# jhtonyKoo/music_mixing_style_transfer

Hardware: AMD Instinct MI355X
Metric: stereo 44.1 kHz segments/sec (FXencoder+MixFXcloner fwd) (higher is better)
Workload: dtype bf16

## Files before the change

include/mst_hip.h:

```cpp
#ifndef MST_HIP_H
#define MST_HIP_H

#include <stddef.h>
#include <stdint.h>

#ifdef __cplusplus
extern "C" {
#endif

typedef enum {
    MST_OK = 0,
    MST_ERR_ARG = -1,
    MST_ERR_UNSUPPORTED = -2,
    MST_ERR_HIP = -3,
    MST_ERR_STATE = -4,
    MST_ERR_WORKSPACE = -5
} MstStatus;

typedef enum {
    MST_PREC_F32 = 0,
    MST_PREC_BF16 = 1,
    MST_PREC_BF16X3 = 2
} MstPrecision;

#define MST_MAX_BLOCKS 32

int mst_version(void);
const char *mst_last_error(void);

typedef struct MstTcn MstTcn;

typedef struct {
    int nblocks;
    int ninputs;
    int noutputs;
    int channels;
    int kernel_size;
    int cond_dim;
    int dilations[MST_MAX_BLOCKS];
    int causal;
} MstTcnDesc;

int mst_tcn_create(const MstTcnDesc *desc, MstTcn **out);
int mst_tcn_destroy(MstTcn *tcn);

int mst_tcn_load_block(MstTcn *tcn, int n, const float *conv_w, const float *bn_weight, const float *bn_bias,
                       const float *bn_mean, const float *bn_var, float bn_eps, const float *film_w,
                       const float *film_b, const float *res_w, void *stream);
int mst_tcn_load_output(MstTcn *tcn, const float *w, const float *b, void *stream);

int mst_tcn_set_cond(MstTcn *tcn, const float *cond_dev, int n_rows, long block_stride, void *stream);

size_t mst_tcn_workspace_bytes(const MstTcn *tcn, int B, int L, int precision);

int mst_tcn_forward(MstTcn *tcn, const float *x_dev, float *y_dev, int B, int L, int precision,
                    void *workspace, size_t workspace_bytes, void *stream);
int mst_tcn_forward_blocks(MstTcn *tcn, const float *x_dev, float *act_dev, int B, int L, int precision, int n_run,
                           void *workspace, size_t workspace_bytes, void *stream);

int mst_tcn_set_tuning(MstTcn *tcn, int flags);
int mst_tcn_get_tuning(const MstTcn *tcn, int *flags, int *last_forward_fused_block0);

int mst_tcn_timing_begin(MstTcn *tcn, int max_forwards);
int mst_tcn_timing_end(MstTcn *tcn, float *ms_out, int *n_forwards);

int mst_calib_mainloop(int launches, float *ms_per_launch, float *sclk_mhz, void *stream);

typedef struct MstEnc MstEnc;

typedef struct {
    int nblocks;
    int channels[MST_MAX_BLOCKS + 1];
    int kernels[MST_MAX_BLOCKS];
    int strides[MST_MAX_BLOCKS];
    int dilations[MST_MAX_BLOCKS];
    int valid_padding;
    float act_slope;
} MstEncDesc;

int mst_enc_create(const MstEncDesc *desc, MstEnc **out);
int mst_enc_destroy(MstEnc *enc);
int mst_enc_load_conv(MstEnc *enc, int block, int which, const float *w, const float *bias,
                      const float *bn_weight, const float *bn_bias, const float *bn_mean, const float *bn_var,
                      float bn_eps, void *stream);
int mst_enc_set_tuning(MstEnc *enc, long rows_min_tiles);
int mst_enc_set_schedule(MstEnc *enc, int flags);
int mst_global_avgpool(const float *x_dev, float *y_dev, long rows, int L, void *stream);
int mst_enc_zero_stuff(const float *x_dev, float *y_dev, long rows, long L, int stride, long pad_left, long Lu, void *stream);
size_t mst_enc_workspace_bytes(const MstEnc *enc, int B, int L);
int mst_enc_forward(MstEnc *enc, const float *x_dev, float *emb_dev, int B, int L, int precision, void *workspace,
                    size_t workspace_bytes, void *stream);
int mst_enc_forward_blocks(MstEnc *enc, const float *x_dev, float *out_dev, int B, int L, int precision, int n_run,
                           void *workspace, size_t workspace_bytes, void *stream);
int mst_enc_conv_length(const MstEnc *enc, int block, int which, int L);
int mst_enc_forward_conv(MstEnc *enc, int block, int which, const float *x_dev, float *y_dev, int B, int L, void *stream);
int mst_enc_block_length(const MstEnc *enc, int block, int L);

int mst_film_forward(const float *w_dev, const float *b_dev, const float *cond_dev, int rows, int cond_dim, int C,
                     const float *x_dev, float *y_dev, int B, long L, float *table_dev, void *stream);

int mst_embedding_mean(const float *emb_dev, int n_rows, int dim, float *out_dev, void *stream);

#define MST_SUMSQ_SLOTS 64
#define MST_FX_FORM_EQ_LANE_APPLY 1
#define MST_FX_FORM_EQ_VALU_ENDS 2
#define MST_FX_FORM_COMP_SLICE_SMALL 4
typedef struct {
    unsigned struct_size;
    int forms;
    const double *in_scale_dev;
    double *out_sumsq_dev;
    const double *in_sumsq_dev;
    int post_rms;
    float post_gain;
// ... 150 lines not shown
```

music_mixing_style_transfer_amd/_lib.py:

```python
import ctypes as C
import os

import torch

_HERE = os.path.dirname(os.path.abspath(__file__))
LIB_PATH = os.path.join(_HERE, "csrc", "libmst_hip.so")

MST_OK = 0
MST_PREC_F32 = 0
MST_PREC_BF16 = 1
MST_PREC_BF16X3 = 2
MST_MAX_BLOCKS = 32
TCN_TUNING_DEFAULT = 245
PRECISIONS = {"fp32": MST_PREC_F32, "f32": MST_PREC_F32, "bf16": MST_PREC_BF16, "bf16x3": MST_PREC_BF16X3}

STATUS_NAMES = {0: "MST_OK", -1: "MST_ERR_ARG", -2: "MST_ERR_UNSUPPORTED", -3: "MST_ERR_HIP", -4: "MST_ERR_STATE",
                -5: "MST_ERR_WORKSPACE"}


class MstTcnDesc(C.Structure):
    _fields_ = [("nblocks", C.c_int), ("ninputs", C.c_int), ("noutputs", C.c_int), ("channels", C.c_int),
                ("kernel_size", C.c_int), ("cond_dim", C.c_int), ("dilations", C.c_int * MST_MAX_BLOCKS), ("causal", C.c_int)]


FX_FORM_EQ_LANE_APPLY, FX_FORM_EQ_VALU_ENDS, FX_FORM_COMP_SLICE_SMALL = 1, 2, 4


class MstFxFuse(C.Structure):
    _fields_ = [("struct_size", C.c_uint), ("forms", C.c_int), ("in_scale_dev", C.c_void_p), ("out_sumsq_dev", C.c_void_p),
                ("in_sumsq_dev", C.c_void_p), ("post_rms", C.c_int), ("post_gain", C.c_float), ("out_in_sumsq_dev", C.c_void_p),
                ("out_ms_dev", C.c_void_p), ("in_ms_dev", C.c_void_p)]

    def __init__(self, in_scale_dev=None, out_sumsq_dev=None, in_sumsq_dev=None, post_rms=0, post_gain=0.0, out_in_sumsq_dev=None,
                 out_ms_dev=None, in_ms_dev=None, forms=0):
        super().__init__(C.sizeof(MstFxFuse), forms, in_scale_dev, out_sumsq_dev, in_sumsq_dev, post_rms, post_gain, out_in_sumsq_dev,
                         out_ms_dev, in_ms_dev)


FX_COMP_SPLIT_SERIAL, FX_COMP_TIME_PARALLEL, FX_COMP_WAVE_SERIAL = 0, 1, 2


class MstFxBiquadItemsPlan(C.Structure):
    _fields_ = [("struct_size", C.c_uint), ("M", C.c_int), ("tables_offset", C.c_size_t), ("item_stride", C.c_size_t), ("powers_offset", C.c_size_t),
                ("coef_offset", C.c_size_t), ("total_bytes", C.c_size_t)]

    def __init__(self, *a, **kw):
        super().__init__(*a, **kw)
        self.struct_size = C.sizeof(MstFxBiquadItemsPlan)


class MstFxBiquadPlan(C.Structure):
    _fields_ = [("struct_size", C.c_uint), ("time_parallel", C.c_int), ("M", C.c_int), ("scan_threads", C.c_int), ("record_doubles", C.c_int),
                ("nchunks", C.c_long), ("ends_offset", C.c_size_t), ("starts_offset", C.c_size_t)]

    def __init__(self):
        super().__init__(C.sizeof(MstFxBiquadPlan))


class MstFxCompressorPlan(C.Structure):
    _fields_ = [("struct_size", C.c_uint), ("form", C.c_int), ("nslices", C.c_int), ("record_doubles", C.c_int), ("nchunks", C.c_long),
                ("nbatch", C.c_long), ("ntiles", C.c_long), ("kappa", C.c_double), ("kappa_limit", C.c_double), ("xl_offset", C.c_size_t),
                ("maps_offset", C.c_size_t), ("ystart_offset", C.c_size_t), ("tab_offset", C.c_size_t), ("carry_offset", C.c_size_t),
                ("tsums_offset", C.c_size_t), ("total_bytes", C.c_size_t)]

    def __init__(self):
        super().__init__(C.sizeof(MstFxCompressorPlan))


class MstEncDesc(C.Structure):
    _fields_ = [("nblocks", C.c_int), ("channels", C.c_int * (MST_MAX_BLOCKS + 1)), ("kernels", C.c_int * MST_MAX_BLOCKS),
                ("strides", C.c_int * MST_MAX_BLOCKS), ("dilations", C.c_int * MST_MAX_BLOCKS), ("valid_padding", C.c_int), ("act_slope", C.c_float)]


MST_MSS_MAX_SCALES = 8
MSS_MODES = {"midside": 0, "ori": 1}
MSS_WINDOWS = {"hann": 0, "hamming": 1}


class MstMssDesc(C.Structure):
    _fields_ = [("struct_size", C.c_uint), ("mode", C.c_int), ("n_scales", C.c_int), ("n_fft", C.c_int * MST_MSS_MAX_SCALES),
                ("hop", C.c_int * MST_MSS_MAX_SCALES), ("win_length", C.c_int * MST_MSS_MAX_SCALES), ("window", C.c_int),
                ("eps", C.c_double)]

    def __init__(self, mode=0, n_fft=(), hop=(), win_length=(), window=0, eps=1e-7):
        super().__init__()
        self.struct_size, self.mode, self.n_scales, self.window, self.eps = C.sizeof(MstMssDesc), mode, len(n_fft), window, eps
        for i in range(min(len(n_fft), MST_MSS_MAX_SCALES)):
            self.n_fft[i], self.hop[i], self.win_length[i] = n_fft[i], hop[i], win_length[i]


_P = C.c_void_p
_F = C.c_void_p

SIGNATURES = {
    "mst_version": (C.c_int, []),
    "mst_last_error": (C.c_char_p, []),
    "mst_tcn_create": (C.c_int, [C.POINTER(MstTcnDesc), C.POINTER(_P)]),
    "mst_tcn_destroy": (C.c_int, [_P]),
    "mst_tcn_load_block": (C.c_int, [_P, C.c_int, _F, _F, _F, _F, _F, C.c_float, _F, _F, _F, _P]),
    "mst_tcn_load_output": (C.c_int, [_P, _F, _F, _P]),
    "mst_tcn_set_cond": (C.c_int, [_P, _F, C.c_int, C.c_long, _P]),
    "mst_tcn_workspace_bytes": (C.c_size_t, [_P, C.c_int, C.c_int, C.c_int]),
    "mst_tcn_forward": (C.c_int, [_P, _F, _F, C.c_int, C.c_int, C.c_int, _P, C.c_size_t, _P]),
    "mst_tcn_forward_blocks": (C.c_int, [_P, _F, _F, C.c_int, C.c_int, C.c_int, C.c_int, _P, C.c_size_t, _P]),
    "mst_tcn_set_tuning": (C.c_int, [_P, C.c_int]),
    "mst_tcn_get_tuning": (C.c_int, [_P, C.POINTER(C.c_int), C.POINTER(C.c_int)]),
    "mst_tcn_timing_begin": (C.c_int, [_P, C.c_int]),
    "mst_tcn_timing_end": (C.c_int, [_P, C.POINTER(C.c_float), C.POINTER(C.c_int)]),
    "mst_calib_mainloop": (C.c_int, [C.c_int, C.POINTER(C.c_float), C.POINTER(C.c_float), _P]),
    "mst_enc_create": (C.c_int, [C.POINTER(MstEncDesc), C.POINTER(_P)]),
    "mst_enc_destroy": (C.c_int, [_P]),
    "mst_enc_load_conv": (C.c_int, [_P, C.c_int, C.c_int, _F, _F, _F, _F, _F, _F, C.c_float, _P]),
    "mst_enc_set_tuning": (C.c_int, [_P, C.c_long]),
    "mst_enc_set_schedule": (C.c_int, [_P, C.c_int]),
    "mst_global_avgpool": (C.c_int, [_F, _F, C.c_long, C.c_int, _P]),
    "mst_enc_zero_stuff": (C.c_int, [_F, _F, C.c_long, C.c_long, C.c_int, C.c_long, C.c_long, _P]),
    "mst_enc_workspace_bytes": (C.c_size_t, [_P, C.c_int, C.c_int]),
    "mst_enc_forward": (C.c_int, [_P, _F, _F, C.c_int, C.c_int, C.c_int, _P, C.c_size_t, _P]),
    "mst_enc_forward_blocks": (C.c_int, [_P, _F, _F, C.c_int, C.c_int, C.c_int, C.c_int, _P, C.c_size_t, _P]),
    "mst_enc_block_length": (C.c_int, [_P, C.c_int, C.c_int]),
    "mst_enc_conv_length": (C.c_int, [_P, C.c_int, C.c_int, C.c_int]),
    "mst_enc_forward_conv": (C.c_int, [_P, C.c_int, C.c_int, _F, _F, C.c_int, C.c_int, _P]),
    "mst_film_forward": (C.c_int, [_F, _F, _F, C.c_int, C.c_int, C.c_int, _F, _F, C.c_int, C.c_long, _F, _P]),
    "mst_embedding_mean": (C.c_int, [_F, C.c_int, C.c_int, _F, _P]),
    "mst_fx_biquad_scratch_bytes": (C.c_size_t, [C.c_int, C.c_long, C.c_int, C.c_int]),
    "mst_fx_biquad_plan": (C.c_int, [C.c_int, C.c_long, C.c_int, C.c_int, C.POINTER(MstFxBiquadPlan)]),
    "mst_fx_biquad_tables": (C.c_int, [C.POINTER(C.c_double), C.c_int, C.c_int, C.POINTER(C.c_double), C.POINTER(C.c_double)]),
    "mst_fx_compressor_plan": (C.c_int, [C.c_int, C.c_long, C.c_int, C.c_double, C.c_double, C.c_double, C.c_int, C.POINTER(MstFxCompressorPlan)]),
    "mst_fx_biquad_cascade": (C.c_int, [_F, _F, C.c_int, C.c_long, C.c_int, C.POINTER(C.c_double), C.c_int, _P, C.c_size_t, _P, _P]),
    "mst_fx_biquad_items_scratch_bytes": (C.c_size_t, [C.c_int, C.c_long, C.c_int, C.c_int]),
    "mst_fx_biquad_items_plan": (C.c_int, [C.c_int, C.c_long, C.c_int, C.c_int, C.POINTER(MstFxBiquadItemsPlan)]),
    "mst_fx_biquad_cascade_items": (C.c_int, [_F, _F, C.c_int, C.c_long, C.c_int, _P, C.c_int, _P, C.c_size_t, _P, _P]),
    "mst_fx_compressor_items_table_bytes": (C.c_size_t, [C.c_int]),
    "mst_fx_compressor_items_prepare": (C.c_int, [_P, C.c_int, C.c_long, C.c_int, C.c_double, C.c_int, _P, C.c_size_t, C.POINTER(C.c_int)]),
    "mst_fx_compressor_items": (C.c_int, [_F, _F, C.c_int, C.c_long, C.c_int, _P, _P, C.c_size_t, _P, _P]),
    "mst_fx_midside_imager_items": (C.c_int, [_F, _F, C.c_int, C.c_long, _P, _P, _P, _P, _P]),
    "mst_fx_gain_items": (C.c_int, [_F, _F, C.c_int, C.c_long, C.c_int, _P, _P, _P, _P]),
    "mst_fx_sumsq": (C.c_int, [_F, C.c_int, C.c_long, _P, _P]),
    "mst_fx_rms_pending": (C.c_int, [_P, _P, C.c_long, _P, C.c_long, _P, C.c_int, _P]),
    "mst_fx_scale_items": (C.c_int, [_F, _F, C.c_int, C.c_long, _P, _P]),
    "mst_fx_compressor_scratch_bytes": (C.c_size_t, [C.c_int, C.c_long, C.c_int]),
    "mst_fx_compressor": (C.c_int, [_F, _F, C.c_int, C.c_long, C.c_int, C.c_double, C.c_double, C.c_double, C.c_double,
                                    C.c_double, _P, C.c_size_t, _P, _P]),
    "mst_fx_midside_imager": (C.c_int, [_F, _F, C.c_int, C.c_long, C.c_double, _P, _P, _P]),
    "mst_fx_gain": (C.c_int, [_F, _F, C.c_int, C.c_long, C.c_int, C.c_double, C.c_int, _P, _P]),
    "mst_fx_haas": (C.c_int, [_F, _F, C.c_int, C.c_long, C.c_int, C.c_long, C.c_double, C.c_int, _P]),
    "mst_fx_panner": (C.c_int, [_F, _F, C.c_int, C.c_long, C.c_int, C.c_float, C.c_float, _P]),
    "mst_fx_rms_normalize": (C.c_int, [_F, _F, C.c_int, C.c_long, C.c_long, _P, _P]),
    "mst_fx_convolver_create": (C.c_int, [C.c_long, C.c_long, C.c_int, C.c_int, C.POINTER(_P)]),
    "mst_fx_convolver_destroy": (None, [_P]),
    "mst_fx_convolver_workspace_bytes": (C.c_size_t, [_P]),
    "mst_fx_compressor_grid": (C.c_int, [_F, _F, C.c_int, C.c_long, C.c_int, _F, _F, C.c_double, C.c_double, C.c_double, _P, C.c_size_t,
                                         _P, _P]),
    "mst_fx_range_reduce": (C.c_int, [_F, C.c_long, C.c_int, C.c_int, _P, _P, _P, C.c_int, C.c_int, _P, _P]),
    "mst_fx_onset_hfc": (C.c_int, [_F, C.c_int, C.c_long, C.c_int, C.c_int, C.c_int, _F, _P]),
    "mst_fx_stft_create": (C.c_int, [C.c_long, C.c_long, C.POINTER(C.c_float), C.c_int, C.POINTER(_P)]),
    "mst_fx_stft_destroy": (None, [_P]),
    "mst_fx_stft_workspace_bytes": (C.c_size_t, [_P]),
    "mst_fx_stft_mean_magnitude": (C.c_int, [_P, _F, C.c_long, C.c_int, C.c_int, _F, _P, C.c_size_t, _P]),
# ... 94 lines not shown
```

music_mixing_style_transfer_amd/csrc/mst_api.hip:

```cpp
#include "mst_host.h"

namespace {
thread_local std::string g_err;
}

int mst_fail(int code, const std::string &msg) {
    g_err = msg;
    return code;
}

extern "C" int mst_version(void) { return 103; }
extern "C" const char *mst_last_error(void) { return g_err.c_str(); }
```

music_mixing_style_transfer_amd/csrc/mst_tcn.hip:

```cpp
#include "mst_host.h"
#include "tcn_kernels.h"

struct MstTcnBlock {
    void *w_bf16 = nullptr;
    void *w_x3 = nullptr;
    float *w_f32 = nullptr;
    float *shift = nullptr;
    float *res = nullptr;
    bool loaded = false;
};

struct TcnTuning {
    int flags;
    bool x3_small_tiles() const { return flags & 1; }
    bool bf16_cm() const { return ((flags >> 1) & 3) == 2; }
    bool bf16_fuse0() const { return bf16_cm() && (flags & 32); }
    bool x3_half_cm() const { return flags & 64; }
    bool bf16_whole() const { return bf16_cm() && (flags & 128); }
};

constexpr int TCN_FILM_ROWS0 = 64;
struct MstTcn {
    MstTcnDesc d;
    bool generic = false;
    std::vector<MstEncConv> gconv;
    std::vector<MstTcnBlock> blk;
    float *film_w = nullptr;
    float *film_b = nullptr;
    float *film = nullptr;
    int film_rows = 0, film_cap = 0;
    std::vector<float *> film_retired;
    float *out_w = nullptr, *out_b = nullptr;
    bool out_loaded = false;
    void *zero_row = nullptr;
    int tuning = 245;
    int last_fused0 = 0;
    std::vector<hipEvent_t> ev;
    int ev_max = 0, ev_used = 0;
};


extern "C" int mst_tcn_create(const MstTcnDesc *desc, MstTcn **out) {
    if (!desc || !out) return fail(MST_ERR_ARG, "mst_tcn_create: null argument");
    const MstTcnDesc &d = *desc;
    if (d.nblocks < 1 || d.nblocks > MST_MAX_BLOCKS) return fail(MST_ERR_ARG, "mst_tcn_create: nblocks out of range");
    if (d.channels < 1 || d.kernel_size < 1 || d.ninputs < 1 || d.noutputs < 1 || d.cond_dim < 1)
        return fail(MST_ERR_ARG, "mst_tcn_create: bad layer description");
    if (d.channels % d.ninputs != 0)
        return fail(MST_ERR_UNSUPPORTED, "mst_tcn_create: channel_width must be a multiple of ninputs (grouped 1x1 residual)");
    const bool fast = d.channels == 128 && d.kernel_size == 15 && d.ninputs == 2 && d.noutputs <= 2 && d.dilations[0] == 1 && !d.causal;
    for (int n = 0; n < d.nblocks; ++n)
        if (d.dilations[n] < 1) return fail(MST_ERR_ARG, "mst_tcn_create: dilation < 1");
    MstTcn *t = new MstTcn();
    t->d = d;
    t->generic = !fast;
    t->blk.resize(d.nblocks);
    if (t->generic) {
        t->gconv.resize(d.nblocks + 1);
        for (int n = 0; n < d.nblocks; ++n) {
            const int span = (d.kernel_size - 1) * d.dilations[n];
            const int pad_l = d.causal ? span : span / 2;
            conv_geometry(t->gconv[n], n == 0 ? d.ninputs : d.channels, d.channels, d.kernel_size, 1, d.dilations[n], pad_l, span - pad_l);
        }
        conv_geometry(t->gconv[d.nblocks], d.channels, d.noutputs, 1, 1, 1, 0, 0);
    }
    const size_t fw = (size_t)d.nblocks * 2 * d.channels * d.cond_dim;
    if (hipMalloc((void **)&t->film_w, fw * sizeof(float)) != hipSuccess ||
        hipMalloc((void **)&t->film_b, (size_t)d.nblocks * 2 * d.channels * sizeof(float)) != hipSuccess ||
        hipMalloc(&t->zero_row, 1024) != hipSuccess || hipMemset(t->zero_row, 0, 1024) != hipSuccess ||
        hipMalloc((void **)&t->film, (size_t)d.nblocks * TCN_FILM_ROWS0 * 2 * d.channels * sizeof(float)) != hipSuccess) {
        (void)hipFree(t->film_w);
        (void)hipFree(t->film_b);
        (void)hipFree(t->zero_row);
        (void)hipFree(t->film);
        delete t;
        return fail(MST_ERR_HIP, "mst_tcn_create: hipMalloc failed");
    }
    t->film_cap = TCN_FILM_ROWS0;
    *out = t;
    return MST_OK;
}

extern "C" int mst_tcn_destroy(MstTcn *t) {
    if (!t) return MST_OK;
    for (auto &b : t->blk) {
        (void)hipFree(b.w_bf16);
        (void)hipFree(b.w_x3);
        (void)hipFree(b.w_f32);
        (void)hipFree(b.shift);
        (void)hipFree(b.res);
// ... 265 lines not shown

int tcn_launch_block(const TcnBlockPlan &p, const TcnBlockArgs &a, void *stream) {
    for (const TcnBlockKernel &k : TCN_BLOCK_KERNELS)
        if (k.family == p.family && k.P == p.P && k.tile == p.tile && k.form == p.form && k.block0 == p.block0 &&
            (k.head == p.head || p.family != TCN_BF16)) {
            MST_LAUNCH(k.kernel, dim3((unsigned)p.grid), dim3(256), stream, a);
            MST_CHECK_LAUNCH(k.name);
            return MST_OK;
        }
    return fail(MST_ERR_STATE, "mst_tcn_forward: no block kernel of this tile form (with the fused head the whole-sequence 256-time tile exists at "
                               "sixteen phases only)");
}

int tcn_run_generic(MstTcn *t, const float *x, float *y, float *act_out, int B, int L, int n_run, void *ws, void *stream) {
    const int C = t->d.channels;
    const size_t buf_bytes = align_up((size_t)B * L * C * sizeof(float), 256);
    float *buf[2] = {(float *)ws, (float *)((unsigned char *)ws + buf_bytes)};
    const float *cur = x;
    int rc, pp = 0;
    for (int n = 0; n < n_run; ++n) {
        float *dst = (act_out && n == n_run - 1) ? act_out : buf[pp];
        const int cin = n == 0 ? t->d.ninputs : C;
        if ((rc = tcn_launch_generic(t->gconv[n], cur, dst, B, L, 1, t->film + (size_t)n * t->film_rows * 2 * C, t->film_rows,
                                     t->blk[n].res, C / cin, stream)))
            return rc;
        cur = dst;
        pp ^= 1;
    }
    if (act_out) return MST_OK;
    return tcn_launch_generic(t->gconv[t->d.nblocks], cur, y, B, L, 2, nullptr, 1, nullptr, 1, stream);
}

int tcn_run(MstTcn *t, const float *x, float *y, float *act_out, int B, int L, int precision, int n_run, void *ws,
            size_t ws_bytes, void *stream) {
    if (!t || !x || B < 1 || L < 1) return fail(MST_ERR_ARG, "mst_tcn_forward: bad argument");
    if (precision != MST_PREC_F32 && precision != MST_PREC_BF16 && precision != MST_PREC_BF16X3)
        return fail(MST_ERR_ARG, "mst_tcn_forward: bad precision");
    for (auto &b : t->blk)
        if (!b.loaded) return fail(MST_ERR_STATE, "mst_tcn_forward: block weights not loaded");
    if (!t->out_loaded) return fail(MST_ERR_STATE, "mst_tcn_forward: output conv not loaded");
    if (t->film_rows == 0) return fail(MST_ERR_STATE, "mst_tcn_forward: mst_tcn_set_cond has not been called");
    if (t->film_rows != 1 && t->film_rows != B)
        return fail(MST_ERR_ARG, "mst_tcn_forward: condition rows must be 1 or equal the batch size");
    const size_t need = mst_tcn_workspace_bytes(t, B, L, precision);
    if (!ws || ws_bytes < need) return fail(MST_ERR_WORKSPACE, "mst_tcn_forward: workspace too small");
    if (t->generic) return tcn_run_generic(t, x, y, act_out, B, L, n_run, ws, stream);
    const int nblocks = t->d.nblocks;
    TcnBlockPlan plan[MST_MAX_BLOCKS] = {};
    for (int n = 1; n < n_run; ++n) {
        plan[n] = tcn_plan_block(t->tuning, precision, t->d.dilations[n], L, B, !act_out && n == nblocks - 1,
                                 n == 1 && nblocks > 2 && t->d.dilations[0] == 1);
        if (plan[n].grid > 0x7fffffffL) return fail(MST_ERR_ARG, "mst_tcn_forward: grid too large");
    }
    const size_t buf_bytes = align_up((size_t)B * L * 128 * tcn_elem(precision), 256);
    unsigned char *buf[2] = {(unsigned char *)ws, (unsigned char *)ws + buf_bytes};
    const int Lp = L;
    hipEvent_t *ev = nullptr;
    if (!act_out && t->ev_used < t->ev_max) {
        ev = t->ev.data() + (size_t)t->ev_used * (nblocks + 2);
        t->ev_used++;
        MST_HIP_TRY(hipEventRecord(ev[0], (hipStream_t)stream));
    }

    const bool fuse0 = plan[1].block0;
    t->last_fused0 = fuse0 ? 1 : 0;
    if (!fuse0) {
        TcnBlock0Args a;
        a.x = x;
        a.y = buf[0];
        a.w = t->blk[0].w_f32;
        a.shift = t->blk[0].shift;
        a.film = t->film;
        a.res = t->blk[0].res;
        a.film_rows = t->film_rows;
        a.B = B;
        a.L = L;
        a.Lp = Lp;
        a.wpk16 = t->blk[0].w_bf16;
        if (precision == MST_PREC_BF16)
            MST_LAUNCH(tcn_block0_mfma_kernel, dim3(B * ((L + 255) / 256)), dim3(256), stream, a);
        else
            MST_LAUNCH((tcn_block0_kernel<float>), dim3(B * ((L + 511) / 512)), dim3(256), stream, a);
        MST_CHECK_LAUNCH("tcn_block0_kernel");
    }
    if (ev) MST_HIP_TRY(hipEventRecord(ev[1], (hipStream_t)stream));
    int cur = 0;
    for (int n = 1; n < n_run; ++n) {
        const TcnBlockPlan &p = plan[n];
        TcnBlockArgs a;
        a.x = buf[cur];
        a.y = buf[cur ^ 1];
        a.wpk = precision == MST_PREC_BF16 ? t->blk[n].w_bf16 : (precision == MST_PREC_BF16X3 ? t->blk[n].w_x3 : (void *)t->blk[n].w_f32);
        a.shift = t->blk[n].shift;
        a.film = t->film + (size_t)n * t->film_rows * 256;
        a.res = t->blk[n].res;
        a.film_rows = t->film_rows;
        a.B = B;
        a.L = L;
        a.Lp = Lp;
        a.d = t->d.dilations[n];
        a.tiles_phase = p.tiles_phase;
        a.tiles_step = p.tiles_step;
        a.out_w = t->out_w;
        a.out_b = t->out_b;
        a.y_out = p.head ? y : nullptr;
        a.nout = t->d.noutputs;
        a.xcd_tiles = p.xcd_tiles;
        a.zeros = t->zero_row;
        if (p.block0) {
            a.x0 = x;
            a.w0pk = t->blk[0].w_bf16;
            a.shift0 = t->blk[0].shift;
            a.film0 = t->film;
            a.res0 = t->blk[0].res;
        }
        int rc;
        if ((rc = tcn_launch_block(p, a, stream))) return rc;
        if (ev) MST_HIP_TRY(hipEventRecord(ev[n + 1], (hipStream_t)stream));
        cur ^= 1;
    }
    if (act_out) {
        const size_t total = (size_t)B * L * 128;
        const unsigned grid = (unsigned)((total + 255) / 256);
        if (precision == MST_PREC_BF16)
            MST_LAUNCH((tcn_unpack_kernel<__bf16>), dim3(grid), dim3(256), stream, (const void *)buf[cur], act_out, B, L, Lp);
        else
            MST_LAUNCH((tcn_unpack_kernel<float>), dim3(grid), dim3(256), stream, (const void *)buf[cur], act_out, B, L, Lp);
        MST_CHECK_LAUNCH("tcn_unpack_kernel");
        return MST_OK;
    }
    if (!plan[nblocks - 1].head) {
        TcnOutArgs o;
        o.x = buf[cur];
        o.y = y;
        o.w = t->out_w;
        o.bias = t->out_b;
        o.nout = t->d.noutputs;
        o.B = B;
        o.L = L;
        o.Lp = Lp;
        const int grid = B * ((L + 63) / 64);
        if (precision == MST_PREC_BF16)
            MST_LAUNCH((tcn_output_kernel<__bf16>), dim3(grid), dim3(256), stream, o);
        else
            MST_LAUNCH((tcn_output_kernel<float>), dim3(grid), dim3(256), stream, o);
        MST_CHECK_LAUNCH("tcn_output_kernel");
    }
    if (ev) MST_HIP_TRY(hipEventRecord(ev[nblocks + 1], (hipStream_t)stream));
    return MST_OK;
}

}

extern "C" int mst_tcn_set_tuning(MstTcn *t, int flags) {
    if (!t) return fail(MST_ERR_ARG, "mst_tcn_set_tuning: null handle");
    const int form = (flags >> 1) & 3;
    if (flags < 0 || flags > 255 || (form != 0 && form != 2) || ((flags >> 3) & 1) || (form == 2 && !((flags >> 4) & 1)))
        return fail(MST_ERR_ARG, "mst_tcn_set_tuning: unknown flag bits (bits 1-2 = 0 or 2, form 2 with bit 4, no bit 3: the kernels the others "
                                 "selected left the library)");
    t->tuning = flags;
    return MST_OK;
}

extern "C" int mst_tcn_get_tuning(const MstTcn *t, int *flags, int *last_forward_fused_block0) {
    if (!t) return fail(MST_ERR_ARG, "mst_tcn_get_tuning: null handle");
    if (flags) *flags = t->tuning;
    if (last_forward_fused_block0) *last_forward_fused_block0 = t->last_fused0;
    return MST_OK;
}

extern "C" int mst_tcn_timing_begin(MstTcn *t, int max_forwards) {
    if (!t || max_forwards < 1) return fail(MST_ERR_ARG, "mst_tcn_timing_begin: bad argument");
    for (auto e : t->ev) (void)hipEventDestroy(e);
    t->ev.assign((size_t)max_forwards * (t->d.nblocks + 2), nullptr);
    for (auto &e : t->ev) MST_HIP_TRY(hipEventCreate(&e));
    t->ev_max = max_forwards;
    t->ev_used = 0;
    return MST_OK;
}

extern "C" int mst_tcn_timing_end(MstTcn *t, float *ms_out, int *n_forwards) {
    if (!t || !ms_out || !n_forwards) return fail(MST_ERR_ARG, "mst_tcn_timing_end: bad argument");
    const int per = t->d.nblocks + 2;
    for (int k = 0; k <= t->d.nblocks; ++k) ms_out[k] = 0.0f;
    for (int f = 0; f < t->ev_used; ++f) {
        MST_HIP_TRY(hipEventSynchronize(t->ev[(size_t)f * per + per - 1]));
        for (int k = 0; k <= t->d.nblocks; ++k) {
            float ms = 0.0f;
            MST_HIP_TRY(hipEventElapsedTime(&ms, t->ev[(size_t)f * per + k], t->ev[(size_t)f * per + k + 1]));
            ms_out[k] += ms;
        }
    }
    if (t->ev_used > 0)
        for (int k = 0; k <= t->d.nblocks; ++k) ms_out[k] /= (float)t->ev_used;
    *n_forwards = t->ev_used;
    for (auto e : t->ev) (void)hipEventDestroy(e);
    t->ev.clear();
    t->ev_max = t->ev_used = 0;
    return MST_OK;
}

extern "C" int mst_calib_mainloop(int launches, float *ms_per_launch, float *sclk_mhz, void *stream) {
    if (launches < 2 || !ms_per_launch || !sclk_mhz) return fail(MST_ERR_ARG, "mst_calib_mainloop: bad argument");
    constexpr int WG = 512, REP = 32;
    const size_t wbytes = (size_t)120 * 256 * 16;
    void *w = nullptr;
    float *out = nullptr;
    long long *clk = nullptr;
    hipEvent_t e0 = nullptr, e1 = nullptr;
    int rc = MST_OK;
    auto cleanup = [&]() {
        if (w) (void)hipFree(w);
        if (out) (void)hipFree(out);
        if (clk) (void)hipFree(clk);
        if (e0) (void)hipEventDestroy(e0);
        if (e1) (void)hipEventDestroy(e1);
    };
#define MST_CALIB_TRY(x)                                                        \
    if ((x) != hipSuccess) {                                                    \
        rc = fail(MST_ERR_HIP, "mst_calib_mainloop: HIP call failed");          \
        cleanup();                                                              \
        return rc;                                                              \
    }
    MST_CALIB_TRY(hipMalloc(&w, wbytes));
    MST_CALIB_TRY(hipMalloc((void **)&out, (size_t)WG * 256 * sizeof(float)));
    MST_CALIB_TRY(hipMalloc((void **)&clk, 2 * sizeof(long long)));
    MST_CALIB_TRY(hipEventCreate(&e0));
    MST_CALIB_TRY(hipEventCreate(&e1));
    MST_LAUNCH(tcn_calib_fill_kernel, dim3((unsigned)(wbytes / 4 + 255) / 256), dim3(256), stream, (unsigned *)w, (int)(wbytes / 4));
    const int warm = launches / 2, timed = launches - warm;
    for (int i = 0; i < warm; ++i) MST_LAUNCH(tcn_calib_mainloop_kernel, dim3(WG), dim3(256), stream, (const void *)w, out, clk, REP);
    MST_CALIB_TRY(hipEventRecord(e0, (hipStream_t)stream));
    for (int i = 0; i < timed; ++i) MST_LAUNCH(tcn_calib_mainloop_kernel, dim3(WG), dim3(256), stream, (const void *)w, out, clk, REP);
    MST_CALIB_TRY(hipEventRecord(e1, (hipStream_t)stream));
    MST_CALIB_TRY(hipEventSynchronize(e1));
    float ms = 0.0f;
    MST_CALIB_TRY(hipEventElapsedTime(&ms, e0, e1));
    long long c[2] = {0, 0};
    MST_CALIB_TRY(hipMemcpy(c, clk, sizeof(c), hipMemcpyDeviceToHost));
#undef MST_CALIB_TRY
    *ms_per_launch = ms / (float)timed;
    *sclk_mhz = c[1] > 0 ? (float)((double)c[0] / ((double)c[1] / 100.0)) : 0.0f;
    cleanup();
    return MST_OK;
// ... 44 lines not shown
```

music_mixing_style_transfer_amd/csrc/tcn_kernels.h:

```cpp
#pragma once
#include <type_traits>

#include "mst_dev.h"

struct TcnBlockArgs {
    const void *x;
    void *y;
    const void *wpk;
    const float *shift;
    const float *film;
    const float *res;
    int film_rows;
    int B, L, Lp, d;
    int tiles_phase;
    int tiles_step;
    const float *out_w;
    const float *out_b;
    float *y_out;
    int nout;
    const void *zeros;
    int xcd_tiles;
    const float *x0 = nullptr;
    const void *w0pk = nullptr;
    const float *shift0 = nullptr, *film0 = nullptr, *res0 = nullptr;
// ... 384 lines not shown
        const unsigned char *srcp = smem + prow * 256 + ((slot ^ (prow & 15)) << 4);
#pragma unroll
        for (int i = 0; i < T / 16; ++i) {
            if (t < a.L) *(bf16x8 *)dstp = *(const bf16x8 *)(srcp + i * 4096);
            t += dt;
            dstp += dt * 128;
        }
    }
}

template <int P, int NU, bool LAST, int NUMAX>
__device__ __forceinline__ void tcn_reuse_class(f32x4 (&acc)[2][16], bf16x8 (&A0)[NUMAX][2], bf16x8 (&A1)[NUMAX][2], bf16x8 (&ring)[4],
                                                const unsigned char *sm, const MstStream16 &wst, unsigned aoff, int c, int cn, int l16, int g) {
    constexpr int NW = 15 + NU, NCLS = 16 / P;
    static_assert(NW >= 4, "the ring is four windows deep");
    const int rsw = (P * c + l16) & 15, rswn = (P * cn + l16) & 15;
    const unsigned char *rowb = sm + (P * c + l16) * 256, *rowbn = sm + (P * cn + l16) * 256;
#pragma unroll
    for (int kk = 0; kk < 4; ++kk) {
        bf16x8 (&cur)[NUMAX][2] = (kk & 1) ? A1 : A0;
        bf16x8 (&nxt)[NUMAX][2] = (kk & 1) ? A0 : A1;
#pragma unroll
        for (int u = 0; u < NUMAX; ++u) {
            if (kk < 3 && u >= NU) continue;
            if (LAST && kk == 3) continue;
            int j = (kk < 3 ? c : cn) + NCLS * u;
            j = j < 15 ? j : 14;
            const unsigned so = (unsigned)(j * 4 + (kk < 3 ? kk + 1 : 0)) * 8192u;
            nxt[u][0] = __builtin_bit_cast(bf16x8, mst_stream_load16(wst, aoff, so));
            nxt[u][1] = __builtin_bit_cast(bf16x8, mst_stream_load16(wst, aoff + 4096u, so));
        }
#pragma unroll
        for (int i = 0; i < NW; ++i) {
            const int n = kk * NW + i;
            const bf16x8 b = ring[n & 3];
#pragma unroll
            for (int u = 0; u < NU; ++u) {
                const int q = i - u;
                if (q >= 0 && q < 16) {
                    acc[0][q] = __builtin_amdgcn_mfma_f32_16x16x32_bf16(cur[u][0], b, acc[0][q], 0, 0, 0);
                    acc[1][q] = __builtin_amdgcn_mfma_f32_16x16x32_bf16(cur[u][1], b, acc[1][q], 0, 0, 0);
                }
            }
            const int n2 = n + 4, k2 = n2 / NW, i2 = n2 % NW;
            if (k2 < 4)
                ring[n & 3] = *(const bf16x8 *)(rowb + (((4 * k2 + g) ^ rsw) << 4) + i2 * 4096);
            else if (!LAST)
                ring[n & 3] = *(const bf16x8 *)(rowbn + ((g ^ rswn) << 4) + i2 * 4096);
            __builtin_amdgcn_sched_barrier(0);
        }
    }
}

template <int P, int NU, bool LASTC, int NUMAX, int NC>
__device__ __forceinline__ void tcn_reuse_class_x3(f32x4 (&acc)[2][NC], bf16x8 (&H0)[NUMAX][2], bf16x8 (&L0)[NUMAX][2], bf16x8 (&H1)[NUMAX][2],
                                                   bf16x8 (&L1)[NUMAX][2], bf16x8 (&rh)[4], bf16x8 (&rl)[4], const unsigned char *sm_hi,
                                                   const unsigned char *sm_lo, const unsigned char *wbase, size_t lo_img, unsigned aoff, int c, int cn,
                                                   int l16, int g) {
    constexpr int NW = NC - 1 + NU, NCLS = 16 / P;
    static_assert(NW >= 4, "the ring is four windows deep");
    const int rsw = (P * c + l16) & 15, rswn = (P * cn + l16) & 15;
    const int rowb = (P * c + l16) * 256, rowbn = (P * cn + l16) * 256;
#pragma unroll
    for (int kk = 0; kk < 4; ++kk) {
        bf16x8 (&ch)[NUMAX][2] = (kk & 1) ? H1 : H0;
        bf16x8 (&cl)[NUMAX][2] = (kk & 1) ? L1 : L0;
        bf16x8 (&nh)[NUMAX][2] = (kk & 1) ? H0 : H1;
        bf16x8 (&nl)[NUMAX][2] = (kk & 1) ? L0 : L1;
        if (!(LASTC && kk == 3)) {
#pragma unroll
            for (int u = 0; u < NUMAX; ++u) {
                if (kk < 3 && u >= NU) continue;
                int j = (kk < 3 ? c : cn) + NCLS * u;
                j = j < 15 ? j : 14;
                const size_t so = (size_t)((j * 4 + (kk < 3 ? kk + 1 : 0)) * 2) * 4096 + aoff;
#pragma unroll
                for (int m = 0; m < 2; ++m) {
                    nh[u][m] = *(const bf16x8 *)(wbase + so + (size_t)m * 4096);
                    nl[u][m] = *(const bf16x8 *)(wbase + lo_img + so + (size_t)m * 4096);
                }
            }
        }
#pragma unroll
        for (int i = 0; i < NW; ++i) {
            const int n = kk * NW + i;
            const bf16x8 bh = rh[n & 3], bl = rl[n & 3];
#pragma unroll
            for (int u = 0; u < NU; ++u) {
                const int q = i - u;
                if (q >= 0 && q < NC) {
#pragma unroll
                    for (int m = 0; m < 2; ++m) acc[m][q] = __builtin_amdgcn_mfma_f32_16x16x32_bf16(cl[u][m], bh, acc[m][q], 0, 0, 0);
#pragma unroll
                    for (int m = 0; m < 2; ++m) acc[m][q] = __builtin_amdgcn_mfma_f32_16x16x32_bf16(ch[u][m], bl, acc[m][q], 0, 0, 0);
#pragma unroll
                    for (int m = 0; m < 2; ++m) acc[m][q] = __builtin_amdgcn_mfma_f32_16x16x32_bf16(ch[u][m], bh, acc[m][q], 0, 0, 0);
                }
            }
            const int n2 = n + 4, k2 = n2 / NW, i2 = n2 % NW;
            if (k2 < 4) {
                const int ofs = rowb + (((4 * k2 + g) ^ rsw) << 4) + i2 * 4096;
                rh[n & 3] = *(const bf16x8 *)(sm_hi + ofs);
                rl[n & 3] = *(const bf16x8 *)(sm_lo + ofs);
            } else if (!LASTC) {
                const int ofs = rowbn + ((g ^ rswn) << 4) + i2 * 4096;
                rh[n & 3] = *(const bf16x8 *)(sm_hi + ofs);
// ... 915 lines not shown
```

music_mixing_style_transfer_amd/networks/architectures.py:

```python
import ctypes as C
import inspect
import os

import torch
import torch.nn as nn

from .. import _lib
from .network_utils import Conv1d_layer, ConvBlock, FiLM, Res_ConvBlock, _DeviceState


class _HParams(dict):

    def __getattr__(self, k):
        try:
            return self[k]
        except KeyError:
            raise AttributeError(k) from None

    def __setattr__(self, k, v):
        self[k] = v


def _stream_ptr(t):
    return _lib.lib().stream_ptr(t)
# ... 264 lines not shown
        names, _, _, values = inspect.getargvalues(frame)
        self.hparams = _HParams({n: values[n] for n in names if n not in ("self", "frame")})
        self.blocks = nn.ModuleList()
        out_ch = None
        for n in range(nblocks):
            in_ch = out_ch if n > 0 else ninputs
            out_ch = in_ch * channel_growth if channel_growth > 1 else channel_width
            dilation = dilation_growth ** (n % stack_size)
            self.blocks.append(TCNBlock(in_ch, out_ch, kernel_size=kernel_size, dilation=dilation,
                                        padding="same" if causal else "valid", causal=causal, cond_dim=cond_dim,
                                        grouped=grouped, conditional=True if nparams > 0 else False))
        self.output = nn.Conv1d(out_ch, noutputs, kernel_size=1)
        self.precision = os.environ.get("MST_TCN_PRECISION", "fp32")
        self._handle = None
        self._lib = None
        self._sig = None
        self._ws = _Workspace()

    def compute_receptive_field(self):
        hp = self.hparams
        rf = hp.kernel_size
        for n in range(1, hp.nblocks):
            rf += (hp.kernel_size - 1) * hp.dilation_growth ** (n % hp.stack_size)
        return rf

    @staticmethod
    def add_model_specific_args(parent_parser):
        from argparse import ArgumentParser
        parser = ArgumentParser(parents=[parent_parser], add_help=False)
        for name, default in (("ninputs", 1), ("noutputs", 1), ("nblocks", 4), ("kernel_size", 5), ("dilation_growth", 10),
                              ("channel_growth", 1), ("channel_width", 32), ("stack_size", 10)):
            parser.add_argument("--" + name, type=int, default=default)
        for name in ("grouped", "causal", "skip_connections"):
            parser.add_argument("--" + name, default=False, action="store_true")
        return parser

    def _ensure(self, b):
        sig = _signature(self)
        if self._handle is not None and sig == self._sig and self._lib is b:
            return
        self._close()
        hp = self.hparams
        if not hp.nparams > 0:
            raise AttributeError("'TCNBlock' object has no attribute 'film'")
        d = _lib.MstTcnDesc()
        held = list(self.blocks)[-1:] if hp.channel_growth > 1 else list(self.blocks)
        d.nblocks, d.ninputs, d.noutputs = len(held), held[0].in_ch, hp.noutputs
        d.channels, d.kernel_size, d.cond_dim, d.causal = held[-1].out_ch, hp.kernel_size, hp.cond_dim, int(bool(hp.causal))
        for n, blk in enumerate(held):
            d.dilations[n] = blk.dilation
        h = C.c_void_p()
        b.check(b.mst_tcn_create(C.byref(d), C.byref(h)), "mst_tcn_create")
        self._handle, self._lib = h, b
        f = lambda t: t.detach().to("cpu", torch.float32).contiguous()
        for n, blk in enumerate(held):
            _load_tcn_block(b, h, n, blk)
        ow, ob = f(self.output.weight), f(self.output.bias)
        b.check(b.mst_tcn_load_output(h, ow.data_ptr(), ob.data_ptr(), None), "mst_tcn_load_output")
        self._sig = sig

    def _close(self):
        if self._handle is not None:
            self._lib.mst_tcn_destroy(self._handle)
            self._handle = None

    def __del__(self):
        try:
            self._close()
        except Exception:
            pass

    def _set_cond(self, b, x, cond):
        hp = self.hparams
        if isinstance(cond, (list, tuple)):
            if len(cond) != hp.nblocks:
                raise ValueError("TCNModel.forward: a condition list needs one entry per block")
            if hp.channel_growth > 1:
                cond = cond[-1:]
            c = torch.stack([ci.to(x.device, torch.float32) for ci in cond], 0).contiguous()
            rows, stride = c.shape[1], c.shape[1] * c.shape[2]
        else:
            c = cond.to(x.device, torch.float32).contiguous()
            rows, stride = c.shape[0], 0
        if c.shape[-1] != hp.cond_dim:
            raise ValueError(f"TCNModel.forward: condition length {c.shape[-1]} != cond_dim {hp.cond_dim}")
        if rows not in (1, x.shape[0]):
            raise RuntimeError(f"The size of tensor a ({rows}) must match the size of tensor b ({x.shape[0]}) at "
                               f"non-singleton dimension 0")
        b.check(b.mst_tcn_set_cond(self._handle, c.data_ptr(), rows, stride, _stream_ptr(x)), "mst_tcn_set_cond")
        return c

    def forward(self, x, cond):
        return self._run(x, cond, None)

    def forward_blocks(self, x, cond, n_run):
        return self._run(x, cond, n_run)

    def _run(self, x, cond, n_run):
        b = _check_device(x, "TCNModel.forward")
        with b.device_ctx(x):
            return self._run_on(b, x, cond, n_run)

    def _run_on(self, b, x, cond, n_run):
        hp = self.hparams
        if x.dim() != 3 or x.shape[1] != hp.ninputs:
            raise ValueError(f"TCNModel.forward: expected [B, {hp.ninputs}, L], got {tuple(x.shape)}")
# ... 28 lines not shown
```

Baseline: 1801.

## Fuse last three bf16 TCN blocks and output head into one kernel

Adds a tail kernel that runs the final three dilated TCN blocks, with dilations d, 2d and 4d, plus the output projection in one launch. Each workgroup loads a single input tile with a halo, and intermediate activations stay in LDS between blocks. This removes two launches and the global-memory round trips of the intermediate activations. The cost is a larger halo load per tile and extra LDS pressure, and it applies only when the block plans match a strict pattern. Python enables it by default, and the per-block timing report averages the fused blocks.

```diff
diff --git a/include/mst_hip.h b/include/mst_hip.h
--- a/include/mst_hip.h
+++ b/include/mst_hip.h
@@ -60,6 +60,9 @@
 
 int mst_tcn_set_tuning(MstTcn *tcn, int flags);
 int mst_tcn_get_tuning(const MstTcn *tcn, int *flags, int *last_forward_fused_block0);
+
+int mst_tcn_set_fusion(MstTcn *tcn, int flags);
+int mst_tcn_get_fusion(const MstTcn *tcn, int *flags, int *last_forward_fused_tail);
 
 int mst_tcn_timing_begin(MstTcn *tcn, int max_forwards);
 int mst_tcn_timing_end(MstTcn *tcn, float *ms_out, int *n_forwards);
diff --git a/music_mixing_style_transfer_amd/_lib.py b/music_mixing_style_transfer_amd/_lib.py
--- a/music_mixing_style_transfer_amd/_lib.py
+++ b/music_mixing_style_transfer_amd/_lib.py
@@ -12,6 +12,7 @@
 MST_PREC_BF16X3 = 2
 MST_MAX_BLOCKS = 32
 TCN_TUNING_DEFAULT = 245
+TCN_FUSION_DEFAULT = 1
 PRECISIONS = {"fp32": MST_PREC_F32, "f32": MST_PREC_F32, "bf16": MST_PREC_BF16, "bf16x3": MST_PREC_BF16X3}
 
 STATUS_NAMES = {0: "MST_OK", -1: "MST_ERR_ARG", -2: "MST_ERR_UNSUPPORTED", -3: "MST_ERR_HIP", -4: "MST_ERR_STATE",
@@ -105,6 +106,8 @@
     "mst_tcn_forward_blocks": (C.c_int, [_P, _F, _F, C.c_int, C.c_int, C.c_int, C.c_int, _P, C.c_size_t, _P]),
     "mst_tcn_set_tuning": (C.c_int, [_P, C.c_int]),
     "mst_tcn_get_tuning": (C.c_int, [_P, C.POINTER(C.c_int), C.POINTER(C.c_int)]),
+    "mst_tcn_set_fusion": (C.c_int, [_P, C.c_int]),
+    "mst_tcn_get_fusion": (C.c_int, [_P, C.POINTER(C.c_int), C.POINTER(C.c_int)]),
     "mst_tcn_timing_begin": (C.c_int, [_P, C.c_int]),
     "mst_tcn_timing_end": (C.c_int, [_P, C.POINTER(C.c_float), C.POINTER(C.c_int)]),
     "mst_calib_mainloop": (C.c_int, [C.c_int, C.POINTER(C.c_float), C.POINTER(C.c_float), _P]),
diff --git a/music_mixing_style_transfer_amd/csrc/mst_api.hip b/music_mixing_style_transfer_amd/csrc/mst_api.hip
--- a/music_mixing_style_transfer_amd/csrc/mst_api.hip
+++ b/music_mixing_style_transfer_amd/csrc/mst_api.hip
@@ -9,5 +9,5 @@
     return code;
 }
 
-extern "C" int mst_version(void) { return 103; }
+extern "C" int mst_version(void) { return 104; }
 extern "C" const char *mst_last_error(void) { return g_err.c_str(); }
diff --git a/music_mixing_style_transfer_amd/csrc/mst_tcn.hip b/music_mixing_style_transfer_amd/csrc/mst_tcn.hip
--- a/music_mixing_style_transfer_amd/csrc/mst_tcn.hip
+++ b/music_mixing_style_transfer_amd/csrc/mst_tcn.hip
@@ -35,7 +35,10 @@
     void *zero_row = nullptr;
     int tuning = 245;
     int last_fused0 = 0;
+    int fusion = 0;
+    int last_fused_tail = 0;
     std::vector<hipEvent_t> ev;
+    std::vector<char> ev_tail;
     int ev_max = 0, ev_used = 0;
 };
 
@@ -407,12 +410,25 @@
                                  n == 1 && nblocks > 2 && t->d.dilations[0] == 1);
         if (plan[n].grid > 0x7fffffffL) return fail(MST_ERR_ARG, "mst_tcn_forward: grid too large");
     }
+    bool tail = false;
+    if (precision == MST_PREC_BF16 && !act_out && n_run == nblocks && nblocks >= 4 && (t->fusion & 1)) {
+        const int n0 = nblocks - 3;
+        const int d0 = t->d.dilations[n0];
+        tail = t->d.dilations[n0 + 1] == 2 * d0 && t->d.dilations[n0 + 2] == 4 * d0;
+        for (int k = 0; k < 3; ++k) {
+            const TcnBlockPlan &p = plan[n0 + k];
+            tail = tail && p.family == TCN_BF16 && p.form == 1 && p.tile == 256 && p.P == (4 << k) && p.tiles_step == 1 && !p.block0 &&
+                   p.head == (k == 2) && p.grid == plan[n0].grid;
+        }
+    }
+    t->last_fused_tail = tail ? 1 : 0;
     const size_t buf_bytes = align_up((size_t)B * L * 128 * tcn_elem(precision), 256);
     unsigned char *buf[2] = {(unsigned char *)ws, (unsigned char *)ws + buf_bytes};
     const int Lp = L;
     hipEvent_t *ev = nullptr;
     if (!act_out && t->ev_used < t->ev_max) {
         ev = t->ev.data() + (size_t)t->ev_used * (nblocks + 2);
+        t->ev_tail[t->ev_used] = tail ? 1 : 0;
         t->ev_used++;
         MST_HIP_TRY(hipEventRecord(ev[0], (hipStream_t)stream));
     }
@@ -469,6 +485,23 @@
             a.film0 = t->film;
             a.res0 = t->blk[0].res;
         }
+        if (tail && n == nblocks - 3) {
+            TcnTailArgs ta;
+            ta.a = a;
+            ta.a.y = nullptr;
+            ta.a.y_out = y;
+            for (int k = 0; k < 3; ++k) {
+                ta.wpk[k] = t->blk[n + k].w_bf16;
+                ta.shift[k] = t->blk[n + k].shift;
+                ta.film[k] = t->film + (size_t)(n + k) * t->film_rows * 256;
+                ta.res[k] = t->blk[n + k].res;
+            }
+            MST_LAUNCH(tcn_tail_bf16_kernel, dim3((unsigned)p.grid), dim3(256), stream, ta);
+            MST_CHECK_LAUNCH("tcn_tail_bf16_kernel");
+            if (ev)
+                for (int k = 0; k < 3; ++k) MST_HIP_TRY(hipEventRecord(ev[n + k + 1], (hipStream_t)stream));
+            break;
+        }
         int rc;
         if ((rc = tcn_launch_block(p, a, stream))) return rc;
         if (ev) MST_HIP_TRY(hipEventRecord(ev[n + 1], (hipStream_t)stream));
@@ -524,11 +557,26 @@
     return MST_OK;
 }
 
+extern "C" int mst_tcn_set_fusion(MstTcn *t, int flags) {
+    if (!t) return fail(MST_ERR_ARG, "mst_tcn_set_fusion: null handle");
+    if (flags < 0 || flags > 1) return fail(MST_ERR_ARG, "mst_tcn_set_fusion: unknown flag bits (bit 0: the last three blocks as one launch)");
+    t->fusion = flags;
+    return MST_OK;
+}
+
+extern "C" int mst_tcn_get_fusion(const MstTcn *t, int *flags, int *last_forward_fused_tail) {
+    if (!t) return fail(MST_ERR_ARG, "mst_tcn_get_fusion: null handle");
+    if (flags) *flags = t->fusion;
+    if (last_forward_fused_tail) *last_forward_fused_tail = t->last_fused_tail;
+    return MST_OK;
+}
+
 extern "C" int mst_tcn_timing_begin(MstTcn *t, int max_forwards) {
     if (!t || max_forwards < 1) return fail(MST_ERR_ARG, "mst_tcn_timing_begin: bad argument");
     for (auto e : t->ev) (void)hipEventDestroy(e);
     t->ev.assign((size_t)max_forwards * (t->d.nblocks + 2), nullptr);
     for (auto &e : t->ev) MST_HIP_TRY(hipEventCreate(&e));
+    t->ev_tail.assign((size_t)max_forwards, 0);
     t->ev_max = max_forwards;
     t->ev_used = 0;
     return MST_OK;
@@ -540,11 +588,13 @@
     for (int k = 0; k <= t->d.nblocks; ++k) ms_out[k] = 0.0f;
     for (int f = 0; f < t->ev_used; ++f) {
         MST_HIP_TRY(hipEventSynchronize(t->ev[(size_t)f * per + per - 1]));
-        for (int k = 0; k <= t->d.nblocks; ++k) {
-            float ms = 0.0f;
-            MST_HIP_TRY(hipEventElapsedTime(&ms, t->ev[(size_t)f * per + k], t->ev[(size_t)f * per + k + 1]));
-            ms_out[k] += ms;
-        }
+        float ms[MST_MAX_BLOCKS + 1] = {};
+        for (int k = 0; k <= t->d.nblocks; ++k) MST_HIP_TRY(hipEventElapsedTime(&ms[k], t->ev[(size_t)f * per + k], t->ev[(size_t)f * per + k + 1]));
+        if (t->ev_tail[f]) {
+            const int n0 = t->d.nblocks - 3;
+            ms[n0] = ms[n0 + 1] = ms[n0 + 2] = (ms[n0] + ms[n0 + 1] + ms[n0 + 2]) / 3.0f;
+        }
+        for (int k = 0; k <= t->d.nblocks; ++k) ms_out[k] += ms[k];
     }
     if (t->ev_used > 0)
         for (int k = 0; k <= t->d.nblocks; ++k) ms_out[k] /= (float)t->ev_used;
diff --git a/music_mixing_style_transfer_amd/csrc/tcn_kernels.h b/music_mixing_style_transfer_amd/csrc/tcn_kernels.h
--- a/music_mixing_style_transfer_amd/csrc/tcn_kernels.h
+++ b/music_mixing_style_transfer_amd/csrc/tcn_kernels.h
@@ -460,6 +460,184 @@
     }
 }
 
+struct TcnTailArgs {
+    TcnBlockArgs a;
+    const void *wpk[3];
+    const float *shift[3], *film[3], *res[3];
+};
+
+__device__ __forceinline__ void tcn_tail_acc_init(f32x4 (&acc)[2][16], const float *par, int w, int g) {
+#pragma unroll
+    for (int m = 0; m < 2; ++m) {
+        const f32x4 sh = *(const f32x4 *)(par + 32 * w + 16 * m + 4 * g);
+#pragma unroll
+        for (int q = 0; q < 16; ++q) acc[m][q] = sh;
+    }
+}
+
+template <int ROW_IN, int ROW_OUT, bool ZERO_HALO>
+__device__ __forceinline__ void tcn_tail_hand_over(const f32x4 (&acc)[2][16], unsigned char *smem, const float *par, int tid) {
+    asm volatile("" : "+v"(tid));
+    const int w = tid >> 6, l16 = tid & 15, g = (tid >> 4) & 3;
+    bf16x4 xin[2][16];
+#pragma unroll
+    for (int m = 0; m < 2; ++m) {
+        const int co0 = 32 * w + 16 * m + 4 * g;
+#pragma unroll
+        for (int q = 0; q < 16; ++q) {
+            const int row = 16 * q + l16 + ROW_IN;
+            xin[m][q] = *(const bf16x4 *)(smem + row * 256 + (((co0 >> 3) ^ (row & 15)) << 4) + 2 * (co0 & 7));
+        }
+    }
+    __syncthreads();
+#pragma unroll
+    for (int m = 0; m < 2; ++m) {
+        const int co0 = 32 * w + 16 * m + 4 * g;
+        const f32x4 fr = *(const f32x4 *)(par + 128 + co0);
+        const f32x4 fb = *(const f32x4 *)(par + 256 + co0);
+        const f32x4 rs = *(const f32x4 *)(par + 384 + co0);
+#pragma unroll
+        for (int q = 0; q < 16; ++q) {
+            const int row = 16 * q + l16 + ROW_OUT;
+            const float v4[4] = {acc[m][q][0], acc[m][q][1], acc[m][q][2], acc[m][q][3]};
+            *(bf16x4 *)(smem + row * 256 + (((co0 >> 3) ^ (row & 15)) << 4) + 2 * (co0 & 7)) = tcn_epilogue4(v4, fr, fb, rs, xin[m][q]);
+        }
+    }
+    if constexpr (ZERO_HALO) {
+        static_assert(!ZERO_HALO || ROW_OUT == 8, "rows [0, 8) and [264, 272): 16 rows, one 16-byte slot per thread");
+        const int r = tid >> 4;
+        const bf16x8 z = {};
+        *(bf16x8 *)(smem + (r < 8 ? r : 256 + r) * 256 + ((tid & 15) << 4)) = z;
+    }
+    __syncthreads();
+}
+
+__global__ __launch_bounds__(256, 2) void tcn_tail_bf16_kernel(TcnTailArgs ta) {
+    constexpr int T = 256, R = T + 2 * 3 * 4, NC = 16;
+    __shared__ __attribute__((aligned(16))) unsigned char smem[R * 256];
+    __shared__ __attribute__((aligned(16))) float par[3][4 * 128];
+    const TcnBlockArgs &a = ta.a;
+    const int tid = threadIdx.x, lane = tid & 63, w = tid >> 6;
+    const int l16 = lane & 15, g = lane >> 4;
+
+    const int tile = a.xcd_tiles > 0 ? (int)(blockIdx.x & 7) * a.xcd_tiles + (int)(blockIdx.x >> 3) : (int)blockIdx.x;
+    const int pg = tile % a.tiles_phase;
+    const int b = tile / a.tiles_phase;
+    const int phi0 = pg * 4;
+    {
+        const __bf16 *xb = (const __bf16 *)a.x + (size_t)b * a.Lp * 128;
+        const int slot = tid & 15, prow = tid >> 4;
+        constexpr int NPASS = (R + 15) / 16;
+        const long dt = 4l * a.d;
+        long t = (long)(prow / 4 - 3) * a.d + phi0 + (prow % 4);
+        const __bf16 *src = xb + t * 128 + slot * 8;
+        const __bf16 *zsrc = (const __bf16 *)a.zeros + slot * 8;
+        bf16x8 v[NPASS];
+#pragma unroll
+        for (int i = 0; i < NPASS; ++i) {
+            const bool ok = prow + 16 * i < R && t >= 0 && t < a.L;
+            v[i] = *(const bf16x8 *)(ok ? src : zsrc);
+            t += dt;
+            src += dt * 128;
+        }
+        float pv[3][4];
+#pragma unroll
+        for (int k = 0; k < 3; ++k) {
+            const int pc = tid & 127;
+            const float *frow0 = ta.film[k] + (a.film_rows > 1 ? (size_t)b * 256 : 0);
+            pv[k][0] = ta.shift[k][pc];
+            pv[k][1] = frow0[pc];
+            pv[k][2] = frow0[128 + pc];
+            pv[k][3] = ta.res[k][pc];
+        }
+        unsigned char *dst = smem + prow * 256 + ((slot ^ (prow & 15)) << 4);
+#pragma unroll
+        for (int i = 0; i < NPASS; ++i)
+            if (prow + 16 * i < R) *(bf16x8 *)(dst + i * 4096) = v[i];
+        if (tid < 128) {
+#pragma unroll
+            for (int k = 0; k < 3; ++k) {
+                par[k][tid] = pv[k][0];
+                par[k][128 + tid] = pv[k][1];
+                par[k][256 + tid] = pv[k][2];
+                par[k][384 + tid] = pv[k][3];
+            }
+        }
+    }
+    __syncthreads();
+
+    const unsigned aoff = (unsigned)(w * 64 + lane) * 16u;
+    f32x4 acc[2][NC];
+    tcn_tail_acc_init(acc, par[0], w, g);
+    tcn_class_major_whole_tile<4, NC, 3>(acc, smem, mst_stream16(ta.wpk[0], 60u * 2u * 4096u), aoff, l16, g);
+    tcn_tail_hand_over<12, 8, true>(acc, smem, par[0], (int)(aoff >> 4));
+    tcn_tail_acc_init(acc, par[1], w, g);
+    tcn_class_major_whole_tile<8, NC, 1>(acc, smem, mst_stream16(ta.wpk[1], 60u * 2u * 4096u), aoff, l16, g);
+    tcn_tail_hand_over<8, 0, false>(acc, smem, par[1], (int)(aoff >> 4));
+    tcn_tail_acc_init(acc, par[2], w, g);
+    tcn_class_major_whole_tile<16, NC, 0>(acc, smem, mst_stream16(ta.wpk[2], 60u * 2u * 4096u), aoff, l16, g);
+
+    int tid_e = (int)(aoff >> 4);
+    asm volatile("" : "+v"(tid_e));
+    const int w_e = tid_e >> 6, l16_e = tid_e & 15, g_e = (tid_e >> 4) & 3;
+    bf16x4 xin[2][NC];
+#pragma unroll
+    for (int m = 0; m < 2; ++m) {
+        const int co0 = 32 * w_e + 16 * m + 4 * g_e;
+#pragma unroll
+        for (int q = 0; q < NC; ++q) {
+            const int row = 16 * q + l16_e;
+            xin[m][q] = *(const bf16x4 *)(smem + row * 256 + (((co0 >> 3) ^ (row & 15)) << 4) + 2 * (co0 & 7));
+        }
+    }
+    __syncthreads();
+    float hs0[NC], hs1[NC];
+#pragma unroll
+    for (int q = 0; q < NC; ++q) hs0[q] = hs1[q] = 0.0f;
+#pragma unroll
+    for (int m = 0; m < 2; ++m) {
+        const int co0 = 32 * w_e + 16 * m + 4 * g_e;
+        const f32x4 fr = *(const f32x4 *)(par[2] + 128 + co0);
+        const f32x4 fb = *(const f32x4 *)(par[2] + 256 + co0);
+        const f32x4 rs = *(const f32x4 *)(par[2] + 384 + co0);
+        f32x4 ow0 = *(const f32x4 *)(a.out_w + co0), ow1 = {0.0f, 0.0f, 0.0f, 0.0f};
+        if (a.nout > 1) ow1 = *(const f32x4 *)(a.out_w + 128 + co0);
+#pragma unroll
+        for (int q = 0; q < NC; ++q) {
+            const float v4[4] = {acc[m][q][0], acc[m][q][1], acc[m][q][2], acc[m][q][3]};
+            const bf16x4 out = tcn_epilogue4(v4, fr, fb, rs, xin[m][q]);
+#pragma unroll
+            for (int i = 0; i < 4; ++i) {
+                hs0[q] = fmaf(ow0[i], (float)out[i], hs0[q]);
+                hs1[q] = fmaf(ow1[i], (float)out[i], hs1[q]);
+            }
+        }
+    }
+    float *part = (float *)smem;
+#pragma unroll
+    for (int q = 0; q < NC; ++q) {
+        hs0[q] += __shfl_xor(hs0[q], 16);
+        hs1[q] += __shfl_xor(hs1[q], 16);
+        hs0[q] += __shfl_xor(hs0[q], 32);
+        hs1[q] += __shfl_xor(hs1[q], 32);
+        if (g_e == 0) {
+            part[(w_e * 2 + 0) * T + 16 * q + l16_e] = hs0[q];
+            part[(w_e * 2 + 1) * T + 16 * q + l16_e] = hs1[q];
+        }
+    }
+    __syncthreads();
+#pragma unroll
+    for (int i = 0; i < 2 * T / 256; ++i) {
+        const int idx = tid_e + 256 * i, c = idx / T, o = idx % T;
+        const long t = (long)(o / 4) * a.d + phi0 + (o % 4);
+        if (c < a.nout && t < a.L) {
+            const float v = part[(0 * 2 + c) * T + o] + part[(1 * 2 + c) * T + o] + part[(2 * 2 + c) * T + o] +
+                            part[(3 * 2 + c) * T + o] + a.out_b[c];
+            a.y_out[((size_t)b * a.nout + c) * a.L + t] = fminf(1.0f, fmaxf(-1.0f, v));
+        }
+    }
+}
+
 template <int P, int NU, bool LASTC, int NUMAX, int NC>
 __device__ __forceinline__ void tcn_reuse_class_x3(f32x4 (&acc)[2][NC], bf16x8 (&H0)[NUMAX][2], bf16x8 (&L0)[NUMAX][2], bf16x8 (&H1)[NUMAX][2],
                                                    bf16x8 (&L1)[NUMAX][2], bf16x8 (&rh)[4], bf16x8 (&rl)[4], const unsigned char *sm_hi,
diff --git a/music_mixing_style_transfer_amd/networks/architectures.py b/music_mixing_style_transfer_amd/networks/architectures.py
--- a/music_mixing_style_transfer_amd/networks/architectures.py
+++ b/music_mixing_style_transfer_amd/networks/architectures.py
@@ -340,6 +340,7 @@
         h = C.c_void_p()
         b.check(b.mst_tcn_create(C.byref(d), C.byref(h)), "mst_tcn_create")
         self._handle, self._lib = h, b
+        b.check(b.mst_tcn_set_fusion(h, _lib.TCN_FUSION_DEFAULT), "mst_tcn_set_fusion")
         f = lambda t: t.detach().to("cpu", torch.float32).contiguous()
         for n, blk in enumerate(held):
             _load_tcn_block(b, h, n, blk)
```

After: 1823 (median of 6 runs). 1.01x the previous value.
